# keep-starknet-strange/frieda

Measured on AMD Instinct MI355X. Metric: M31 field-elems/s committed (NTT+FRI+Merkle), higher is better.
Workload: dtype u32

## Files before the change

frieda_amd/csrc/context.cpp:

```cpp
#include <cstring>
#include <cstdlib>
#include <string.h>

#include <cstdio>

#include <algorithm>
#include <mutex>

#include "host.h"

extern char** environ;

namespace frieda {

static constexpr uint32_t IDX_MASK = 0x7fffffffu;

CPoint point_from_index(uint32_t index) {
    static const std::array<CPoint, 31> pow2 = [] {
        std::array<CPoint, 31> t{};
        CPoint cur{CIRCLE_GEN_X, CIRCLE_GEN_Y};
        for (auto& e : t) {
            e = cur;
            cur = cp_double(cur);
        }
        return t;
    }();
    CPoint res{1, 0};
    index &= IDX_MASK;
    for (uint32_t b = 0; index; b++, index >>= 1)
        if (index & 1u) res = cp_add(res, pow2[b]);
    return res;
}

Coset Coset::half_odds(uint32_t log_size) {
    Coset c;
    c.initial = 1u << (31 - (log_size + 2));
    c.step = log_size == 0 ? 0u : (1u << (31 - log_size));
    c.log_size = log_size;
    return c;
}
Coset Coset::doubled() const { return Coset{(initial * 2u) & IDX_MASK, (step * 2u) & IDX_MASK, log_size - 1}; }
uint32_t Coset::index_at(uint32_t i) const { return (initial + (uint32_t)((uint64_t)step * i)) & IDX_MASK; }
CPoint Coset::at(uint32_t i) const { return point_from_index(index_at(i)); }

Coset line_coset(uint32_t n, uint32_t m) {
    Coset c = Coset::half_odds(n - 1);
    while (c.log_size > m) c = c.doubled();
    return c;
}

CodecShape codec_shape(size_t len) {
    CodecShape s;
    s.n_felts = (8 * len + 29) / 30;
    uint32_t e = 2;
    while (((size_t)1 << e) < s.n_felts) e++;
    s.n_padded = (size_t)1 << e;
    s.log_size = e - 2;
    return s;
}

struct KernelTimerImpl {
    struct Span {
        const char* name;
        double alg_bytes;
        hipEvent_t start, stop;
    };
    std::vector<Span> spans;
    std::vector<hipEvent_t> pool;
    size_t used = 0;
    hipEvent_t next() {
        if (used == pool.size()) {
            hipEvent_t e;
            (void)hipEventCreate(&e);
            pool.push_back(e);
        }
        return pool[used++];
    }
    ~KernelTimerImpl() {
        for (auto e : pool) (void)hipEventDestroy(e);
    }
};

namespace k {
void timer_begin(KernelTimer* t, hipStream_t s, const char* name, double alg_bytes) {
    auto* ti = reinterpret_cast<KernelTimerImpl*>(t);
    KernelTimerImpl::Span sp{name, alg_bytes, ti->next(), ti->next()};
    (void)hipEventRecord(sp.start, s);
    ti->spans.push_back(sp);
}
void timer_end(KernelTimer* t, hipStream_t s) {
    auto* ti = reinterpret_cast<KernelTimerImpl*>(t);
    (void)hipEventRecord(ti->spans.back().stop, s);
}
}

k::Launch Ctx::launch() const {
    k::Launch l{stream, reinterpret_cast<k::KernelTimer*>(timer)};
    l.tune = &tuning;
    return l;
}

namespace k {
namespace {
struct KnobDesc {
    const char* name;
    long lo, hi;
    bool (*set)(Tuning&, long);
};
const KnobDesc KNOBS[] = {
    {"FRIEDA_T5_WIDE_LOG", 16, 24, [](Tuning& t, long v) { t.t5_wide_log = (uint32_t)v; return true; }},
    {"FRIEDA_T5_REG3_LOG", 0, 30, [](Tuning& t, long v) { t.t5_reg3_log = (uint32_t)v; return true; }},
    {"FRIEDA_T9_MAX_LOG", 8, 19, [](Tuning& t, long v) { t.t9_max_log = (uint32_t)v; return true; }},
    {"FRIEDA_TOP_MAX_LOG", 9, 11, [](Tuning& t, long v) { t.top_max_log = (uint32_t)v; return true; }},
    {"FRIEDA_NTT_CPW", 1, 4, [](Tuning& t, long v) {
         if (v == 4 && !t.lds_opt_in_ok) return false;
         t.ntt_cpw = (uint32_t)v;
         return true;
     }},
    {"FRIEDA_NTT_CPW_SMALL", 1, 4, [](Tuning& t, long v) { t.ntt_cpw_small = (uint32_t)v; return true; }},
    {"FRIEDA_NTT_REP", 0, 2, [](Tuning& t, long v) { t.ntt_rep = (uint32_t)v; return true; }},
    {"FRIEDA_NTT_NO_CP", 0, 1, [](Tuning& t, long v) { t.ntt_no_cp = v != 0; return true; }},
    {"FRIEDA_NTT_NO_PAD8", 0, 1, [](Tuning& t, long v) { t.ntt_no_pad8 = v != 0; return true; }},
    {"FRIEDA_NTT_PACKED_SRC", 0, 1, [](Tuning& t, long v) { t.ntt_packed_src = v != 0; return true; }},
    {"FRIEDA_NTT_TREE_REG_ONLY", 0, 1, [](Tuning& t, long v) { t.ntt_tree_reg_only = v != 0; return true; }},
    {"FRIEDA_NO_ENCODE_TREE_FUSION", 0, 1, [](Tuning& t, long v) { t.no_encode_tree_fusion = v != 0; return true; }},
    {"FRIEDA_ENCODE_TREE_FUSION_PROVE", 0, 1, [](Tuning& t, long v) { t.encode_tree_fusion_prove = v != 0; return true; }},
    {"FRIEDA_NO_SMALL_FUSED", 0, 1, [](Tuning& t, long v) { t.no_small_fused = v != 0; return true; }},
    {"FRIEDA_UNPACK_TILES", 1, 8, [](Tuning& t, long v) {
         if (v != 1 && v != 2 && v != 4 && v != 8) return false;
         t.unpack_tiles = (uint32_t)v;
         return true;
     }},
    {"FRIEDA_INTT_GENERIC", 0, 1, [](Tuning& t, long v) { t.intt_generic = v != 0; return true; }},
    {"FRIEDA_ERASURE_TREE_MIN_LOG", 6, 32, [](Tuning& t, long v) { t.erasure_tree_min_log = (uint32_t)v; return true; }},
    {"FRIEDA_TAIL_RUN_LOG", 4, 11, [](Tuning& t, long v) { t.tail_run_log = (uint32_t)v; return true; }},
    {"FRIEDA_HOST_DECOMMIT", 0, 1, [](Tuning& t, long v) { t.host_decommit = v != 0; return true; }},
    {"FRIEDA_GATHER_COPY", 0, 1, [](Tuning& t, long v) { t.gather_copy = v != 0; return true; }},
    {"FRIEDA_VERIFY_DEVICE_MIN", 0, 2147483648L, [](Tuning& t, long v) { t.verify_device_min = (uint32_t)v; return true; }},
    {"FRIEDA_VERIFY_SPLIT_MAX", 0, 2147483648L, [](Tuning& t, long v) { t.verify_split_max = (uint32_t)v; return true; }},
    {"FRIEDA_OPEN_SMALL_MAX", 0, 512, [](Tuning& t, long v) { t.open_small_max = (uint32_t)v; return true; }},
    {"FRIEDA_TREE_SKIP_LOG", 10, 40, [](Tuning& t, long v) { t.tree_skip_log = (uint32_t)v; return true; }},
    {"FRIEDA_TREE_SKIP_LONE_LOG", 10, 40, [](Tuning& t, long v) { t.tree_skip_lone_log = (uint32_t)v; return true; }},
    {"FRIEDA_SEEDS_FOLD_GROUP", 0, 64, [](Tuning& t, long v) { t.seeds_fold_group = (uint32_t)v; return true; }},
    {"FRIEDA_TP_MIN_WGS", 0, 1 << 30, [](Tuning& t, long v) { t.tp_min_wgs = (uint32_t)v; return true; }},
    {"FRIEDA_GRIND_FRONT_WGS", 0, 2048, [](Tuning& t, long v) { t.grind_front_wgs = (uint32_t)v; return true; }},
    {"FRIEDA_GRIND_ITERS", 0, 64, [](Tuning& t, long v) { t.grind_iters = (uint32_t)v; return true; }},
    {"FRIEDA_BATCH_BUDGET_MB", 0, 262144, [](Tuning& t, long v) { t.batch_budget_mb = (uint32_t)v; return true; }},
    {"FRIEDA_BATCH_CALLS_PER_CTX", 1, 64, [](Tuning& t, long v) { t.batch_calls_per_ctx = (uint32_t)v; return true; }},
};
}

bool tuning_set(Tuning& t, const char* name, long value) {
    if (!name) return false;
    for (const KnobDesc& k : KNOBS) {
        if (strcmp(k.name, name) == 0) {
            if (value < k.lo || value > k.hi) return false;
            return k.set(t, value);
        }
    }
    return false;
}

static const char* const PROCESS_VARS[] = {"FRIEDA_HIP_LIB", "FRIEDA_RCCL_PATH", "FRIEDA_MULTI_FORCE_RCCL", "FRIEDA_MULTI_NO_PREFETCH",
                                           "FRIEDA_MULTI_NO_NUMA_PIN", "FRIEDA_BENCH_FORCE_DIST", "FRIEDA_BENCH_CPU_THREADS", "FRIEDA_TEST_"};
static void warn_unknown_env_once() {
    static std::once_flag once;
    std::call_once(once, [] {
        for (char** e = ::environ; e && *e; e++) {
            if (strncmp(*e, "FRIEDA_", 7) != 0) continue;
            const char* eq = strchr(*e, '=');
            const size_t len = eq ? (size_t)(eq - *e) : strlen(*e);
            bool known = false;
            for (const KnobDesc& k : KNOBS) known = known || (strlen(k.name) == len && strncmp(k.name, *e, len) == 0);
            for (const char* pv : PROCESS_VARS) known = known || strncmp(pv, *e, strlen(pv)) == 0;
            if (!known) fprintf(stderr, "libfrieda_hip: note: environment variable %.*s is not an option of this library (ignored)\n", (int)len, *e);
        }
    });
}

Tuning tuning_from_env() {
    Tuning t;
    warn_unknown_env_once();
    for (const KnobDesc& k : KNOBS) {
        const char* e = getenv(k.name);
        if (!e) continue;
        char* end = nullptr;
        long v = strtol(e, &end, 10);
        if (end == e) v = 1;
        (void)tuning_set(t, k.name, v);
    }
    return t;
}

const Tuning& tuning_defaults() {
    static const Tuning d;
    return d;
}
}

int Ctx::set_kernel_timing(bool enabled) {
    if (enabled && !timer) timer = new KernelTimerImpl();
    if (!enabled && timer) {
        (void)hipStreamSynchronize(stream);
        delete timer;
        timer = nullptr;
    }
    return FRIEDA_OK;
}

std::string Ctx::kernel_timing_report(bool reset) {
    std::string out = "{\"kernels\": [";
    if (timer) {
        (void)hipStreamSynchronize(stream);
        struct Agg {
            const char* name;
            size_t launches;
            double ms, bytes;
        };
        std::vector<Agg> agg;
        for (auto& sp : timer->spans) {
            float ms = 0.f;
            if (hipEventElapsedTime(&ms, sp.start, sp.stop) != hipSuccess) continue;
            Agg* a = nullptr;
            for (auto& x : agg)
                if (strcmp(x.name, sp.name) == 0) a = &x;
            if (!a) {
                agg.push_back(Agg{sp.name, 0, 0.0, 0.0});
                a = &agg.back();
            }
            a->launches++;
            a->ms += ms;
            a->bytes += sp.alg_bytes;
        }
        bool first = true;
        for (auto& a : agg) {
            char buf[256];
            snprintf(buf, sizeof buf, "%s{\"name\": \"%s\", \"launches\": %zu, \"total_ms\": %.6f, \"alg_bytes\": %.1f}", first ? "" : ", ",
                     a.name, a.launches, a.ms, a.bytes);
            out += buf;
            first = false;
        }
        if (reset) {
            timer->spans.clear();
            timer->used = 0;
        }
    }
    out += "]}";
    return out;
}

int Ctx::fail(int code, const std::string& what) {
    err = what;
    return code;
}
int Ctx::hip_fail(hipError_t e, const char* what) {
    err = std::string(what) + ": " + hipGetErrorString(e);
    return FRIEDA_ERR_HIP;
}

int Ctx::ensure_arena(size_t bytes) {
    if (tuning.test_arena_limit && bytes > tuning.test_arena_limit) {
        err = "workspace of " + std::to_string(bytes) + " B refused by the test limit";
        return FRIEDA_ERR_NOMEM;
    }
    if (bytes <= arena_bytes) return FRIEDA_OK;
    if (arena) {
        FR_HIP(this, hipStreamSynchronize(stream));
        FR_HIP(this, hipFree(arena));
        arena = nullptr;
        arena_bytes = 0;
    }
    size_t want = (bytes + ((size_t)1 << 20) - 1) & ~(((size_t)1 << 20) - 1);
    hipError_t e = hipMalloc((void**)&arena, want);
// ... 103 lines not shown
```

frieda_amd/csrc/kernels.h:

```cpp
#pragma once
#include <hip/hip_runtime.h>
#include <stddef.h>
#include <stdint.h>

#include "field.h"

namespace frieda {
namespace k {

inline size_t tw_level_offset(uint32_t n, uint32_t lv) { return ((size_t)1 << (n - 1)) - ((size_t)1 << (n - 1 - lv)); }
__device__ __forceinline__ size_t tw_level_offset_dev(uint32_t n, uint32_t lv) {
    return ((size_t)1 << (n - 1)) - ((size_t)1 << (n - 1 - lv));
}

struct KernelTimer;
struct Tuning {
    uint32_t t5_wide_log = 18;
    uint32_t t5_reg3_log = 0;
    uint32_t t9_max_log = 17;
    uint32_t top_max_log = 9;
    uint32_t ntt_cpw = 4;
    uint32_t ntt_cpw_small = 1;
    uint32_t ntt_rep = 2;
    bool ntt_no_pad8 = false;
    bool ntt_packed_src = true;
    bool ntt_no_cp = false;
    bool ntt_tree_reg_only = false;
    bool no_encode_tree_fusion = false;
    bool encode_tree_fusion_prove = false;
    bool no_small_fused = false;
    uint32_t unpack_tiles = 4;
    bool intt_generic = false;
    uint32_t erasure_tree_min_log = 15;
    uint32_t tail_run_log = 9;
    bool host_decommit = false;
    bool gather_copy = false;
    uint32_t verify_device_min = 2;
    uint32_t verify_split_max = 256;
    uint32_t open_small_max = 512;
    uint32_t test_grind_first_log = 0;
    uint32_t batch_budget_mb = 0;
    uint32_t tree_skip_log = 18;
    uint32_t tree_skip_lone_log = 23;
    uint32_t tp_min_wgs = 768;
    uint32_t grind_iters = 0;
    uint32_t grind_front_wgs = 768;
    uint32_t seeds_fold_group = 0;
    uint32_t batch_calls_per_ctx = 1;
    uint64_t device_mem_bytes = 0;
    bool lds_opt_in_ok = true;
    uint64_t test_arena_limit = 0;
    uint64_t test_verify_pass_bytes = 0;
    uint64_t test_verify_scratch_bytes = 0;
    bool test_poison = false;
    uint32_t test_poison_word = 0;
};
inline uint32_t tree_skip_threshold(const Tuning& t, uint32_t batch) {
    return batch >= 2 ? t.tree_skip_log : (t.tree_skip_lone_log > t.tree_skip_log ? t.tree_skip_lone_log : t.tree_skip_log);
}
Tuning tuning_from_env();
bool tuning_set(Tuning& t, const char* name, long value);
const Tuning& tuning_defaults();

struct Launch {
    hipStream_t stream;
    KernelTimer* timer;
    uint32_t batch = 1;
    size_t bstride = 0;
    const Tuning* tune = &tuning_defaults();
};
void timer_begin(KernelTimer* t, hipStream_t s, const char* name, double alg_bytes);
void timer_end(KernelTimer* t, hipStream_t s);
struct Scope {
    const Launch& l;
    Scope(const Launch& l_, const char* name, double alg_bytes) : l(l_) {
        if (l.timer) timer_begin(l.timer, l.stream, name, alg_bytes * l.batch);
    }
    ~Scope() {
        if (l.timer) timer_end(l.timer, l.stream);
    }
};

struct DomainScalars {
    uint32_t init_x, init_y;
    uint32_t inv_init_x, inv_init_y;
};

void unpack30(const Launch& L, const uint8_t* d_bytes, size_t len, uint32_t* d_out, size_t n_out, size_t src_bstride = 0);

int blake2s_ceiling(hipStream_t s, uint32_t* d_scratch, double* leaf_per_s, double* node_per_s, double* clock = nullptr);
size_t blake2s_ceiling_scratch_bytes();

void bit_reverse_columns(const Launch& L, uint32_t* d_cols, size_t stride, uint32_t ncols, uint32_t log_size);

struct TwiddleSeeds {
    CPoint p0;
    CPoint step[32];
};
void gen_twiddles(const Launch& L, uint32_t n, const TwiddleSeeds& seeds, uint32_t* d_tw, uint32_t* d_itw, void* d_scratch8k);

void circle_evaluate(const Launch& L_, const uint32_t* d_coef, size_t coef_stride, uint32_t ncols, uint32_t L, uint32_t n,
                     const uint32_t* d_tw, DomainScalars ds, uint32_t* d_out, size_t out_stride);
void circle_evaluate_prefix(const Launch& L_, const uint32_t* d_coef, size_t coef_stride, uint32_t ncols, uint32_t L, uint32_t n, uint32_t out_log,
                            const uint32_t* d_tw, DomainScalars ds, uint32_t* d_out, size_t out_stride);

struct EncodeTreeSink {
    uint8_t* layers;
    uint8_t* last_out;
};
constexpr uint32_t ENCODE_TREE_LEVELS = 7;
hipError_t ntt_opt_in_dynamic_lds();
struct EncodeFoldSink {
    const uint32_t* itw;
    uint32_t alpha0[4], alpha1[4];
    bool accumulate;
    uint32_t* line1;
    uint32_t* line2;
};
bool circle_evaluate_fold2(const Launch& L_, const uint32_t* d_coef, size_t coef_stride, uint32_t L, uint32_t n, const uint32_t* d_tw,
                           DomainScalars ds, uint32_t* d_out, size_t out_stride, const EncodeFoldSink& fs, hipError_t* err);
struct BlobSource {
    const uint8_t* bytes;
    size_t len;
    size_t bstride;
    size_t n_padded;
};
uint32_t circle_evaluate_into_tree(const Launch& L_, const uint32_t* d_coef, size_t coef_stride, uint32_t ncols, uint32_t L, uint32_t n,
                               const uint32_t* d_tw, DomainScalars ds, uint32_t* d_out, size_t out_stride, const EncodeTreeSink* sink,
                               const BlobSource* blob = nullptr);

void circle_interpolate_block(const Launch& L_, const uint32_t* d_block, size_t in_stride, uint32_t ncols, uint32_t L, uint32_t n,
                              uint32_t block, const uint32_t* d_itw, DomainScalars ds, uint32_t* d_coef, size_t out_stride);
void cells_combine(const Launch& L_, const uint32_t* d_w, const uint32_t* d_vinv, uint32_t R, uint32_t ncols, uint32_t m, uint32_t* d_coef,
                   size_t coef_stride, size_t vinv_pitch = 0);
size_t cells_inverse_scratch_bytes(uint32_t R);
uint32_t* cells_inverse_index_buffer(uint8_t* d_scratch, uint32_t R);
void cells_matrix_inverse_device(const Launch& L_, const uint32_t* d_cell_index, uint32_t R, uint32_t j_bits, uint32_t m, uint32_t n,
                                 const uint32_t* d_tw, uint8_t* d_scratch, const uint32_t** d_vinv_out, size_t* pitch_out,
                                 const uint32_t** d_state_out);
void pack30(const Launch& L_, const uint32_t* d_felts, size_t n_felts, uint8_t* d_out, size_t len);

struct ErasureDomain {
    CPoint init;
    CPoint step_pow[32];
    uint32_t n;
};
void erasure_points(const Launch& L_, const ErasureDomain& g, const uint32_t* d_pos, uint32_t count, uint32_t* d_px, uint32_t* d_py);
void erasure_lines(const Launch& L_, const ErasureDomain& g, const uint32_t* d_pos, uint32_t n_lines, uint32_t* d_la, uint32_t* d_lb,
                   uint32_t* d_lc);
size_t erasure_zpart_chunks(uint32_t count, uint32_t n_lines);
void erasure_zeval(const Launch& L_, const uint32_t* d_px, const uint32_t* d_py, uint32_t count, const uint32_t* d_la, const uint32_t* d_lb,
                   const uint32_t* d_lc, uint32_t n_lines, bool own, uint32_t* d_zpart, uint32_t* d_z);
void erasure_known_weights(const Launch& L_, const uint32_t* d_px, const uint32_t* d_py, uint32_t count, uint32_t n, uint32_t* d_z);
void erasure_cellconst(const Launch& L_, const ErasureDomain& g, const uint32_t* d_cell_pos, uint32_t n_cells, uint32_t m, uint32_t* d_kc);
void erasure_zeval_cells(const Launch& L_, const uint32_t* d_px, uint32_t count, uint32_t m, const uint32_t* d_kc, uint32_t n_cells, bool own,
                         uint32_t* d_zpart, uint32_t* d_z);
void erasure_known_weights_cells(const Launch& L_, const uint32_t* d_px, uint32_t count, uint32_t n, uint32_t m, uint32_t* d_z);
size_t erasure_sample_lists_chunks(uint32_t n_cells);
hipError_t erasure_sample_lists(const Launch& L_, const uint32_t* d_idx, uint32_t n_cells, uint32_t domain_cells, uint32_t ncols, uint32_t log_cell,
                          uint32_t* d_owner, uint32_t* d_chunk_sum, uint32_t* d_chunk_off, uint32_t* d_first_cell, uint32_t* d_first_row,
                          uint32_t* d_state, uint32_t* d_pos, uint32_t* d_src);
void erasure_cell_firsts(const Launch& L_, const uint32_t* d_pos, uint32_t n_cells, uint32_t log_cell, uint32_t* d_out);
void erasure_lines32(const Launch& L_, const uint32_t* d_px128, const uint32_t* d_py128, const uint32_t* d_la, const uint32_t* d_lb, const uint32_t* d_lc,
                     uint32_t n_lines, uint32_t nodes, uint32_t* d_out);
void erasure_pairmul(const Launch& L_, const uint32_t* d_ext, uint32_t n_nodes, uint32_t size, uint32_t* d_out);
void erasure_ze(const Launch& L_, const ErasureDomain& g1, const uint32_t* d_zs, uint32_t count, uint32_t n, uint32_t* d_ze);
void erasure_fold_prefix(const Launch& L_, const uint32_t* d_in, size_t in_stride, uint32_t ncols, uint32_t out_log, uint32_t cnt, const uint32_t* d_tw,
                         uint32_t dom_n, uint32_t* d_out, size_t out_stride);
void erasure_gather(const Launch& L_, const uint32_t* d_src, const uint32_t* d_pos, uint32_t count, uint32_t* d_out);
void erasure_scatter(const Launch& L_, const uint32_t* d_cells, const uint32_t* d_src, const uint32_t* d_pos, const uint32_t* d_z, uint32_t count,
                     uint32_t ncols, uint32_t log_cell, uint32_t* d_w, size_t w_stride);
void erasure_divide(const Launch& L_, const uint32_t* d_ev, size_t ev_stride, const uint32_t* d_z, const uint32_t* d_px, uint32_t count, uint32_t ncols,
                    uint32_t n, uint32_t* d_block, size_t block_stride);
void erasure_check(const Launch& L_, const uint32_t* d_cells, const uint32_t* d_src, const uint32_t* d_pos, uint32_t count, uint32_t ncols,
                   uint32_t log_cell, const uint32_t* d_ev, size_t ev_stride, uint32_t* d_mismatch);

// ... 259 lines not shown
```

frieda_amd/csrc/ntt.hip:

```cpp
#include <hip/hip_runtime.h>

#include <type_traits>

#include <cstdlib>

#include "clock_stamps.h"
#include "kernels.h"
#include "tree_dev.h"

namespace frieda {
namespace k {

namespace {
using namespace treedev;

constexpr int NTT_THREADS = 256;
constexpr uint32_t TILE_LOG = 12;
#ifndef FRIEDA_NTT_PAD32
constexpr uint32_t TILE_WORDS = (1u << TILE_LOG) + (1u << (TILE_LOG - 4));
#else
constexpr uint32_t TILE_WORDS = (1u << TILE_LOG) + (1u << (TILE_LOG - 5));
#endif
constexpr uint32_t MAX_COLS_PER_WG = 4;
constexpr uint32_t MID_LOG_W = 4;
// ... 360 lines not shown
            const uint32_t lo = 8 - 4 * s;
            uint32_t* col = lds + pbase[s];
#pragma unroll
            for (int r = 0; r < 16; r++) x[r] = col[pad((uint32_t)r << lo)];
            radix16_stage(x, twd[s]);
            if (s + 1 < NS || LOG_W != 0) {
#pragma unroll
                for (int r = 0; r < 16; r++) col[pad((uint32_t)r << lo)] = x[r];
            }
            if (LOG_W == 0 && NS == 3 && s == 1)
                __builtin_amdgcn_wave_barrier();
            else
                __syncthreads();
        }
        uint32_t* dst = out + (size_t)c * a.out_stride;
        if (LOG_W == 0) {
            uint4* o = reinterpret_cast<uint4*>(dst + gbase + 16u * g);
            o[0] = make_uint4(x[0], x[1], x[2], x[3]);
            o[1] = make_uint4(x[4], x[5], x[6], x[7]);
            o[2] = make_uint4(x[8], x[9], x[10], x[11]);
            o[3] = make_uint4(x[12], x[13], x[14], x[15]);
        } else {
#pragma unroll
            for (int kk = 0; kk < 4; kk++) {
                const uint32_t e = piece_e(kk), p = pad(e);
                *reinterpret_cast<uint4*>(dst + global_of(e)) = make_uint4(lds[p], lds[p + 1], lds[p + 2], lds[p + 3]);
            }
            __syncthreads();
        }
    }
}

struct PackedBlob {
    const uint8_t* p;
    uint32_t full;
    uint32_t tail;
};
__device__ __forceinline__ PackedBlob packed_blob(const uint8_t* __restrict__ p, size_t len) {
    PackedBlob b{p, (uint32_t)(len >> 2), 0u};
    for (size_t i = 4 * (size_t)b.full; i < len; i++) b.tail |= (uint32_t)p[i] << (8 * (i & 3));
    return b;
}
__device__ __forceinline__ uint32_t packed_dword(const PackedBlob& b, uint32_t d) {
    const bool in = d < b.full;
    const uint32_t v = *reinterpret_cast<const uint32_t*>(b.p + ((in ? d : 0u) << 2));
    return in ? v : (d == b.full ? b.tail : 0u);
}
__device__ __forceinline__ uint32_t packed_felt(const PackedBlob& b, uint32_t f) {
    const uint32_t d = (15u * f) >> 4, sh = (30u * f) & 31u;
    const uint64_t pair = ((uint64_t)packed_dword(b, d + 1) << 32) | packed_dword(b, d);
    return (uint32_t)(pair >> sh) & 0x3fffffffu;
}

template <int COLS, bool PACKED>
__global__ __launch_bounds__(NTT_THREADS) void ntt_tile12_rep_kernel(NttArgs a) {
    ntt_enter();
    constexpr int NS = 2;
    constexpr uint32_t LOG_W = MID_LOG_W;
    __shared__ uint32_t lds[TILE_WORDS];
    const uint32_t g = threadIdx.x;
    const uint32_t nwb_log = a.i_lo - LOG_W;
    const uint32_t wblk = blockIdx.x & ((1u << nwb_log) - 1);
    const uint32_t hblk0 = (blockIdx.x >> nwb_log) << a.rep_log;
    constexpr uint32_t wmask = (1u << LOG_W) - 1;
    const size_t col0 = (size_t)blockIdx.y * COLS;
    uint32_t* out = a.out + col0 * a.out_stride + blockIdx.z * a.bstride_w;

    auto piece_e = [&](int kk) { return 4u * g + 1024u * (uint32_t)kk; };
    auto low_of = [&](uint32_t e) { return (wblk << LOG_W) | ((e >> LOG_W) << a.i_lo) | (e & wmask); };

    const uint32_t e0 = stage_group_base(g, 8);
    uint32_t src[COLS][16];
    if constexpr (PACKED) {
        const PackedBlob blob = packed_blob(a.pk + blockIdx.z * a.pk_bstride, a.pk_len);
#pragma unroll
        for (int c = 0; c < COLS; c++) {
#pragma unroll
            for (int r = 0; r < 16; r++) {
                const uint32_t idx = low_of(e0 | ((uint32_t)r << 8)) & a.in_mask;
                const bool ok = idx < a.in_limit;
                const uint32_t v = packed_felt(blob, ok ? (uint32_t)((col0 + c) * a.pk_col_felts) + idx : 0u);
                src[c][r] = ok ? v : 0u;
            }
        }
    } else {
#pragma unroll
        for (int c = 0; c < COLS; c++) {
#pragma unroll
            for (int r = 0; r < 16; r++) {
                const uint32_t idx = low_of(e0 | ((uint32_t)r << 8)) & a.in_mask;
                src[c][r] = idx < a.in_limit ? (a.in + col0 * a.in_stride + blockIdx.z * a.bstride_w)[(size_t)c * a.in_stride + idx] : 0u;
            }
        }
    }
    uint32_t pbase[NS];
#pragma unroll
    for (int s = 0; s < NS; s++) {
        const uint32_t lo = 8 - 4 * s;
        pbase[s] = pad(stage_group_base(g, lo));
    }

#pragma unroll 1
    for (uint32_t h = 0; h < (1u << a.rep_log); h++) {
        const uint32_t hblk = hblk0 + h;
        const uint32_t gbase = hblk << (a.i_hi + 1);
        uint32_t twd[NS][15];
#pragma unroll
        for (int s = 0; s < NS; s++) {
            const uint32_t lo = 8 - 4 * s;
            const uint32_t base = stage_group_base(g, lo);
#pragma unroll
            for (int q = 0; q < 4; q++) {
                const uint32_t b = lo + 3 - q;
                const uint32_t i = a.i_lo + b - LOG_W;
                const uint32_t hbase = (hblk << (a.i_hi - i)) | (base >> (b + 1));
                const uint32_t* lvl = a.tw + tw_level_offset_dev(a.n, i - 1) + hbase;
#pragma unroll
                for (int u = 0; u < (1 << q); u++) {
                    uint32_t v = lvl[u];
                    if (s == 0) v = (uint32_t)__builtin_amdgcn_readfirstlane((int)v);
                    twd[s][(1 << q) - 1 + u] = 2u * v;
                }
            }
        }
#pragma unroll
        for (int c = 0; c < COLS; c++) {
            uint32_t x[16];
#pragma unroll
            for (int r = 0; r < 16; r++) x[r] = src[c][r];
#pragma unroll
            for (int s = 0; s < NS; s++) {
                const uint32_t lo = 8 - 4 * s;
                uint32_t* col = lds + pbase[s];
                if (s > 0) {
#pragma unroll
                    for (int r = 0; r < 16; r++) x[r] = col[pad((uint32_t)r << lo)];
                }
                radix16_stage(x, twd[s]);
#pragma unroll
                for (int r = 0; r < 16; r++) col[pad((uint32_t)r << lo)] = x[r];
                __syncthreads();
            }
            uint32_t* dst = out + (size_t)c * a.out_stride + gbase;
#pragma unroll
            for (int kk = 0; kk < 4; kk++) {
                const uint32_t e = piece_e(kk), p = pad(e);
                *reinterpret_cast<uint4*>(dst + low_of(e)) = make_uint4(lds[p], lds[p + 1], lds[p + 2], lds[p + 3]);
            }
            __syncthreads();
        }
    }
}

struct NttTreeArgs {
    NttArgs a;
    uint8_t* layers;
    uint8_t* last_out;
    size_t bstride;
};


template <bool STORE_ALL>
__device__ __forceinline__ void last_pass_four_columns(const NttArgs& a, uint32_t* lds, uint32_t g, uint32_t hblk, const uint32_t* in, uint32_t* out,
                                                       uint32_t (&v)[4][16]) {
    const uint32_t gbase = hblk << TILE_LOG;
    uint32_t pbase[3];
    uint32_t twd[3][15];
#pragma unroll
    for (int s = 0; s < 3; s++) {
        const uint32_t lo = 8 - 4 * s;
        const uint32_t base = stage_group_base(g, lo);
        pbase[s] = pad(base);
#pragma unroll
        for (int q = 0; q < 4; q++) {
            const uint32_t b = lo + 3 - q;
            const uint32_t hbase = (hblk << (11 - b)) | (base >> (b + 1));
            if (s == 2 && q == 3) {
#pragma unroll
                for (int u = 0; u < 8; u++) twd[s][7 + u] = 2u * circle_twiddle(a.tw, a.n, hbase + (uint32_t)u, a.init_y);
            } else {
                const uint32_t* lvl = a.tw + tw_level_offset_dev(a.n, b - 1) + hbase;
#pragma unroll
                for (int u = 0; u < (1 << q); u++) {
                    uint32_t v = lvl[u];
                    if (s == 0) v = (uint32_t)__builtin_amdgcn_readfirstlane((int)v);
                    twd[s][(1 << q) - 1 + u] = 2u * v;
                }
            }
        }
    }
    auto piece_e = [&](int kk) { return 4u * g + 1024u * (uint32_t)kk; };

    uint4 pre[4];
#pragma unroll
    for (int kk = 0; kk < 4; kk++) pre[kk] = *reinterpret_cast<const uint4*>(in + ((gbase | piece_e(kk)) & a.in_mask));

#pragma unroll
    for (int c = 0; c < 4; c++) {
#pragma unroll
        for (int kk = 0; kk < 4; kk++) {
            const uint32_t p = pad(piece_e(kk));
            lds[p] = pre[kk].x;
            lds[p + 1] = pre[kk].y;
            lds[p + 2] = pre[kk].z;
            lds[p + 3] = pre[kk].w;
        }
        __syncthreads();
        if (c + 1 < 4) {
            const uint32_t* src = in + (size_t)(c + 1) * a.in_stride;
#pragma unroll
            for (int kk = 0; kk < 4; kk++) pre[kk] = *reinterpret_cast<const uint4*>(src + ((gbase | piece_e(kk)) & a.in_mask));
        }
#pragma unroll
        for (int s = 0; s < 3; s++) {
            const uint32_t lo = 8 - 4 * s;
            uint32_t* col = lds + pbase[s];
            uint32_t* x = v[c];
#pragma unroll
            for (int r = 0; r < 16; r++) x[r] = col[pad((uint32_t)r << lo)];
            radix16_stage<FRIEDA_NTT_GROUP_FUSED>(*reinterpret_cast<uint32_t(*)[16]>(x), twd[s]);
            if (s < 2) {
#pragma unroll
                for (int r = 0; r < 16; r++) col[pad((uint32_t)r << lo)] = x[r];
            }
            if (s == 1)
                __builtin_amdgcn_wave_barrier();
            else
                __syncthreads();
        }
        if (STORE_ALL) {
            uint4* o = reinterpret_cast<uint4*>(out + (size_t)c * a.out_stride + gbase + 16u * g);
            o[0] = make_uint4(v[c][0], v[c][1], v[c][2], v[c][3]);
            o[1] = make_uint4(v[c][4], v[c][5], v[c][6], v[c][7]);
            o[2] = make_uint4(v[c][8], v[c][9], v[c][10], v[c][11]);
            o[3] = make_uint4(v[c][12], v[c][13], v[c][14], v[c][15]);
        }
    }

}

FR_CLOCK_DECL(g_clock_ntt_last_tree)
template <bool STORE_ALL, bool REG_ONLY, bool TP>
__global__ __launch_bounds__(NTT_THREADS) void ntt_last_tree_kernel(NttTreeArgs A) {
    ntt_enter();
    __shared__ uint32_t lds[TILE_WORDS];
    __shared__ __attribute__((aligned(16))) uint32_t RC[8 * (256 + 4)];
    __shared__ __attribute__((aligned(16))) uint32_t RD[8 * (128 + 4)];
    const NttArgs& a = A.a;
    uint32_t g_tie = threadIdx.x;
    FR_CLOCK_BEGIN(g_tie)
    const uint32_t g = g_tie;
    const uint32_t hblk = blockIdx.x;
    const uint32_t gbase = hblk << TILE_LOG;
    const uint32_t* in = a.in + blockIdx.z * a.bstride_w;
    uint32_t* out = a.out + blockIdx.z * a.bstride_w;

    uint32_t v[4][16];
    last_pass_four_columns<STORE_ALL>(a, lds, g, hblk, in, out, v);

    const uint32_t m = a.n;
    uint8_t* layers = A.layers + blockIdx.z * A.bstride;
    uint8_t* out_b = STORE_ALL ? layers + layer_off(m, m - 1) : nullptr;
    uint8_t* out_c = STORE_ALL ? layers + layer_off(m, m - 2) : nullptr;
    uint8_t* out_d = STORE_ALL ? layers + layer_off(m, m - 3) : nullptr;
    uint8_t* out_e = STORE_ALL ? layers + layer_off(m, m - 4) : (REG_ONLY ? A.last_out + blockIdx.z * A.bstride : nullptr);
    const size_t leaf0 = (size_t)gbase + 16u * g;
    uint32_t hprev[8], hdprev[8];
#pragma unroll 1
    for (int it = 0; it < 4; it++) {
        const size_t l0 = leaf0 + 4u * (uint32_t)it;
        uint32_t hb[2][8];
        auto half_ab = [&](auto half_c) {
            constexpr int half = decltype(half_c)::value;
            uint32_t ha[2][8];
            leaf_hash<TP ? FRIEDA_B2_IDLE_NTT_LEAF : B2_LAT>(v[0][2 * half], v[1][2 * half], v[2][2 * half], v[3][2 * half], ha[0]);
            leaf_hash<TP ? FRIEDA_B2_IDLE_NTT_LEAF : B2_LAT>(v[0][2 * half + 1], v[1][2 * half + 1], v[2][2 * half + 1], v[3][2 * half + 1], ha[1]);
            uint32_t mm[16];
#pragma unroll
            for (int w = 0; w < 8; w++) mm[w] = ha[0][w], mm[8 + w] = ha[1][w];
            b2_merkle_block<TP ? FRIEDA_B2_IDLE_NTT_NODE : B2_LAT>(mm, hb[half]);
        };
        half_ab(std::integral_constant<int, 0>{});
        half_ab(std::integral_constant<int, 1>{});
        if (STORE_ALL) {
            store_hash(out_b, l0 >> 1, hb[0]);
            store_hash(out_b, (l0 >> 1) + 1, hb[1]);
        }
        uint32_t hc[8];
        {
            uint32_t mm[16];
#pragma unroll
            for (int w = 0; w < 8; w++) mm[w] = hb[0][w], mm[8 + w] = hb[1][w];
            b2_merkle_block<TP ? FRIEDA_B2_IDLE_NTT_NODE : B2_LAT>(mm, hc);
        }
        if (STORE_ALL) store_hash(out_c, l0 >> 2, hc);
        if ((it & 1) == 0) {
#pragma unroll
            for (int w = 0; w < 8; w++) hprev[w] = hc[w];
        } else {
            uint32_t hd[8], mm[16];
#pragma unroll
            for (int w = 0; w < 8; w++) mm[w] = hprev[w], mm[8 + w] = hc[w];
            b2_merkle_block<TP ? FRIEDA_B2_IDLE_NTT_NODE : B2_LAT>(mm, hd);
            if (STORE_ALL) store_hash(out_d, l0 >> 3, hd);
            if (it == 1) {
#pragma unroll
// ... 178 lines not shown
    }
    {
        uint4* o = reinterpret_cast<uint4*>(a.out + (size_t)c * a.out_stride + gbase + 16u * g);
        o[0] = make_uint4(x[0], x[1], x[2], x[3]);
        o[1] = make_uint4(x[4], x[5], x[6], x[7]);
        o[2] = make_uint4(x[8], x[9], x[10], x[11]);
        o[3] = make_uint4(x[12], x[13], x[14], x[15]);
        uint32_t* mine = lds + pad(16u * g);
#pragma unroll
        for (int r = 0; r < 16; r++) mine[r] = x[r];
    }
    __syncthreads();
    const uint32_t T = threadIdx.x, n = a.n;
    const size_t e0 = (size_t)gbase + 4u * T;
    uint32_t v[4][4];
#pragma unroll
    for (int cc = 0; cc < 4; cc++) {
        const uint32_t* t4 = cp_lds + cc * TILE_WORDS + pad(4u * T);
#pragma unroll
        for (int k = 0; k < 4; k++) v[cc][k] = t4[k];
    }
    const QM31Mat am0 = qm_matrix({A.alpha0[0], A.alpha0[1], A.alpha0[2], A.alpha0[3]});
    const QM31Mat am1 = qm_matrix({A.alpha1[0], A.alpha1[1], A.alpha1[2], A.alpha1[3]});
    const size_t i0 = e0 >> 1;
    const uint2 xy = *reinterpret_cast<const uint2*>(A.itw + 2 * (i0 >> 2));
    const uint32_t it0 = (i0 & 2) ? m31_neg(xy.x) : xy.y, it1 = (i0 & 2) ? xy.x : m31_neg(xy.y);
    const uint32_t il = A.itw[e0 >> 2];
    QM31 l1[2];
    l1[0] = qm_fold_pair(QM31{v[0][0], v[1][0], v[2][0], v[3][0]}, QM31{v[0][1], v[1][1], v[2][1], v[3][1]}, it0, am0);
    l1[1] = qm_fold_pair(QM31{v[0][2], v[1][2], v[2][2], v[3][2]}, QM31{v[0][3], v[1][3], v[2][3], v[3][3]}, it1, am0);
    const size_t s1 = (size_t)1 << (n - 1), s2 = (size_t)1 << (n - 2);
    uint32_t* d1 = A.line1 + i0;
    if (ACC) {
        const QM31 al = {A.alpha0[0], A.alpha0[1], A.alpha0[2], A.alpha0[3]};
        const QM31 asq = qm_mul(al, al);
        uint2 o[4];
#pragma unroll
        for (int cc = 0; cc < 4; cc++) o[cc] = *reinterpret_cast<const uint2*>(d1 + cc * s1);
        l1[0] = qm_add(qm_mul(QM31{o[0].x, o[1].x, o[2].x, o[3].x}, asq), l1[0]);
        l1[1] = qm_add(qm_mul(QM31{o[0].y, o[1].y, o[2].y, o[3].y}, asq), l1[1]);
    }
    *reinterpret_cast<uint2*>(d1) = make_uint2(l1[0].a, l1[1].a);
    *reinterpret_cast<uint2*>(d1 + s1) = make_uint2(l1[0].b, l1[1].b);
    *reinterpret_cast<uint2*>(d1 + 2 * s1) = make_uint2(l1[0].c, l1[1].c);
    *reinterpret_cast<uint2*>(d1 + 3 * s1) = make_uint2(l1[0].d, l1[1].d);
    const QM31 l2 = qm_fold_pair(l1[0], l1[1], il, am1);
    uint32_t* d2 = A.line2 + (e0 >> 2);
    d2[0] = l2.a;
    d2[s2] = l2.b;
    d2[2 * s2] = l2.c;
    d2[3 * s2] = l2.d;
}

}

FR_CLOCK_READER(frieda_debug_clock_ntt_last_tree, g_clock_ntt_last_tree)

namespace {
uint32_t evaluate_plan(const Launch& L_, const uint32_t* d_coef, size_t coef_stride, uint32_t ncols, uint32_t L, uint32_t n, uint32_t out_log,
                       const uint32_t* d_tw, DomainScalars ds, uint32_t* d_out, size_t out_stride, const EncodeTreeSink* sink,
                       const EncodeFoldSink* fsink = nullptr, const BlobSource* blob = nullptr);
}

void circle_evaluate(const Launch& L_, const uint32_t* d_coef, size_t coef_stride, uint32_t ncols, uint32_t L, uint32_t n,
                     const uint32_t* d_tw, DomainScalars ds, uint32_t* d_out, size_t out_stride) {
    (void)evaluate_plan(L_, d_coef, coef_stride, ncols, L, n, n, d_tw, ds, d_out, out_stride, nullptr);
}

void circle_evaluate_prefix(const Launch& L_, const uint32_t* d_coef, size_t coef_stride, uint32_t ncols, uint32_t L, uint32_t n, uint32_t out_log,
                            const uint32_t* d_tw, DomainScalars ds, uint32_t* d_out, size_t out_stride) {
    (void)evaluate_plan(L_, d_coef, coef_stride, ncols, L, n, out_log < L ? L : (out_log > n ? n : out_log), d_tw, ds, d_out, out_stride, nullptr);
}

uint32_t circle_evaluate_into_tree(const Launch& L_, const uint32_t* d_coef, size_t coef_stride, uint32_t ncols, uint32_t L, uint32_t n,
                               const uint32_t* d_tw, DomainScalars ds, uint32_t* d_out, size_t out_stride, const EncodeTreeSink* sink,
                               const BlobSource* blob) {
    return evaluate_plan(L_, d_coef, coef_stride, ncols, L, n, n, d_tw, ds, d_out, out_stride, sink, nullptr, blob);
}

hipError_t ntt_opt_in_dynamic_lds() {
    const int bytes = (int)(MAX_COLS_PER_WG * TILE_WORDS * sizeof(uint32_t));
    hipError_t e = hipFuncSetAttribute(reinterpret_cast<const void*>(ntt_tile_kernel), hipFuncAttributeMaxDynamicSharedMemorySize, bytes);
    if (e != hipSuccess) return e;
    e = hipFuncSetAttribute(reinterpret_cast<const void*>(ntt_last_fold_cp_kernel<false>), hipFuncAttributeMaxDynamicSharedMemorySize, bytes);
    if (e != hipSuccess) return e;
    return hipFuncSetAttribute(reinterpret_cast<const void*>(ntt_last_fold_cp_kernel<true>), hipFuncAttributeMaxDynamicSharedMemorySize, bytes);
}

bool circle_evaluate_fold2(const Launch& L_, const uint32_t* d_coef, size_t coef_stride, uint32_t L, uint32_t n, const uint32_t* d_tw,
                           DomainScalars ds, uint32_t* d_out, size_t out_stride, const EncodeFoldSink& fs, hipError_t* err) {
    *err = hipSuccess;
    if (evaluate_plan(L_, d_coef, coef_stride, 4, L, n, n, d_tw, ds, d_out, out_stride, nullptr, &fs)) return true;
    if (!fs.accumulate) {
        *err = hipMemsetAsync(fs.line1, 0, sizeof(uint32_t) * ((size_t)4 << (n - 1)), L_.stream);
        if (*err != hipSuccess) return false;
    }
    fold_circle_into_line(L_, fs.line1, (size_t)1 << (n - 1), d_out, out_stride, n, fs.itw, ds, Alpha{{fs.alpha0[0], fs.alpha0[1], fs.alpha0[2], fs.alpha0[3]}});
    fold_line(L_, fs.line1, (size_t)1 << (n - 1), n - 1, n, fs.itw, ds, Alpha{{fs.alpha1[0], fs.alpha1[1], fs.alpha1[2], fs.alpha1[3]}}, fs.line2,
              (size_t)1 << (n - 2));
    return false;
}

namespace {
uint32_t evaluate_plan(const Launch& L_, const uint32_t* d_coef, size_t coef_stride, uint32_t ncols, uint32_t L, uint32_t n, uint32_t out_log,
                       const uint32_t* d_tw, DomainScalars ds, uint32_t* d_out, size_t out_stride, const EncodeTreeSink* sink,
                       const EncodeFoldSink* fsink, const BlobSource* blob) {
    const size_t N = (size_t)1 << out_log;
    hipStream_t s = L_.stream;
    bool blob_pending = blob != nullptr;
    auto unpack_now = [&]() {
        unpack30(L_, blob->bytes, blob->len, const_cast<uint32_t*>(d_coef), blob->n_padded, blob->bstride);
        blob_pending = false;
    };
    const double enc_bytes = 4.0 * ncols * ((double)N + (double)((size_t)1 << L));
    if (L == 0) {
        if (blob_pending) unpack_now();
        Scope scope(L_, "ntt_broadcast", enc_bytes);
        dim3 grid((unsigned)((N + 255) / 256), ncols, L_.batch);
        ntt_broadcast_kernel<<<grid, 256, 0, s>>>(d_coef, coef_stride, d_out, out_stride, N, L_.bstride / 4);
        return 0;
    }
    const uint32_t cpw_max = L_.tune->ntt_cpw <= MAX_COLS_PER_WG ? L_.tune->ntt_cpw : MAX_COLS_PER_WG;
    uint32_t cpw = cpw_max;
    while (ncols % cpw) cpw--;
    const size_t lds_bytes = (size_t)cpw * TILE_WORDS * sizeof(uint32_t);

    const uint32_t last_t = L < TILE_LOG ? L : TILE_LOG;
    uint32_t rest = L - last_t;
    const uint32_t mid_max = TILE_LOG - MID_LOG_W;
    const uint32_t n_mid_generic = (rest + mid_max - 1) / mid_max;
    uint32_t n_mid_fast = 0;
    NttArgs a{};
    a.in = d_coef;
    a.in_stride = coef_stride;
    a.in_mask = (uint32_t)(((size_t)1 << L) - 1);
    a.out = d_out;
    a.out_stride = out_stride;
    a.tw = d_tw;
    a.n = n;
    a.init_y = ds.init_y;
    a.bstride_w = L_.bstride / 4;
    uint32_t cpw4 = MAX_COLS_PER_WG;
    const uint32_t cpw_small = L_.tune->ntt_cpw_small;
    if ((N >> TILE_LOG) * (size_t)L_.batch < 512) cpw4 = cpw_small;
    while (ncols % cpw4) cpw4--;
    uint32_t fused_levels = 0;
    auto launch_pass = [&](uint32_t t, const char* name) {
        const bool aligned = ((a.in_stride | a.out_stride) & 3) == 0 && (a.in_mask & 3u) == 3u &&
                             ((reinterpret_cast<uintptr_t>(a.in) | reinterpret_cast<uintptr_t>(a.out) | L_.bstride) & 15) == 0;
        const uint32_t hb_log = n - 1 - a.i_hi;
        const uint64_t rep_wgs = (uint64_t)((N >> TILE_LOG) >> (hb_log < 3 ? hb_log : 3)) * (ncols / 2) * L_.batch;
        const bool use_rep = L_.tune->ntt_rep == 1 || (L_.tune->ntt_rep == 2 && rep_wgs >= 1024);
        const bool rep = use_rep && out_log == n && aligned && t == 8 && a.log_w == MID_LOG_W && hb_log >= 1 && ((uint64_t)a.in_mask >> (a.i_hi + 1)) == 0 && ncols % 2 == 0;
        bool packed = false;
        if (blob_pending) {
            packed = rep && L_.tune->ntt_packed_src && blob->len >= 4 && blob->len <= ((size_t)1 << 30) &&
                     (uint64_t)ncols * coef_stride <= ((uint64_t)1 << 28) && (reinterpret_cast<uintptr_t>(blob->bytes) & 3) == 0 &&
                     (L_.batch == 1 || (blob->bstride & 3) == 0);
            if (packed)
                blob_pending = false;
            else
                unpack_now();
        }
        if (sink && aligned && a.log_w == 0 && t == 12 && ncols == 4 && n >= TILE_LOG && out_log == n) {
            NttTreeArgs ta{};
            ta.a = a;
            ta.a.ncols = 4;
            ta.layers = sink->layers;
            ta.last_out = sink->last_out;
            ta.bstride = L_.bstride;
            const bool reg_only = L_.tune->ntt_tree_reg_only;
            const uint32_t levels = reg_only ? 5u : ENCODE_TREE_LEVELS;
            double bytes = enc_bytes / ((n_mid_fast ? n_mid_fast : n_mid_generic) + 1) + 48.0 * (double)N;
            for (uint32_t l = 1; l < levels; l++) bytes += 96.0 * (double)(N >> l);
            Scope scope(L_, reg_only ? "ntt_last_tree5" : "ntt_last_tree7", bytes);
            const dim3 grid((unsigned)(N >> TILE_LOG), 1, L_.batch);
            const bool tp = (size_t)grid.x * grid.z >= L_.tune->tp_min_wgs;
#define FR_LAUNCH_LAST_TREE(SA, RO)                                                      \
    do {                                                                                 \
        if (tp)                                                                          \
            ntt_last_tree_kernel<SA, RO, true><<<grid, NTT_THREADS, 0, s>>>(ta);         \
        else                                                                             \
            ntt_last_tree_kernel<SA, RO, false><<<grid, NTT_THREADS, 0, s>>>(ta);        \
    } while (0)
            if (sink->layers && reg_only)
                FR_LAUNCH_LAST_TREE(true, true);
            else if (sink->layers)
                FR_LAUNCH_LAST_TREE(true, false);
            else if (reg_only)
                FR_LAUNCH_LAST_TREE(false, true);
            else
                FR_LAUNCH_LAST_TREE(false, false);
#undef FR_LAUNCH_LAST_TREE
            fused_levels = levels;
            return;
        }
        if (fsink && aligned && a.log_w == 0 && t == 12 && ncols == 4 && n >= TILE_LOG + 2 && out_log == n && L_.batch == 1 &&
            ((reinterpret_cast<uintptr_t>(fsink->line1) | reinterpret_cast<uintptr_t>(fsink->line2) | reinterpret_cast<uintptr_t>(fsink->itw)) & 15) == 0) {
            NttFoldArgs fa{};
            fa.a = a;
            fa.a.ncols = 4;
            fa.itw = fsink->itw;
            fa.inv_init_y = ds.inv_init_y;
            for (int i = 0; i < 4; i++) fa.alpha0[i] = fsink->alpha0[i], fa.alpha1[i] = fsink->alpha1[i];
            fa.line1 = fsink->line1;
            fa.line2 = fsink->line2;
            Scope scope(L_, "ntt_last_fold2", enc_bytes / ((n_mid_fast ? n_mid_fast : n_mid_generic) + 1) + 36.0 * (double)N);
            const dim3 grid((unsigned)(N >> TILE_LOG), 1, 1);
            const bool side_by_side = (N >> TILE_LOG) < 512 && L_.tune->lds_opt_in_ok && L_.tune->ntt_cpw == 4 && !L_.tune->ntt_no_cp;
            const size_t cp_lds = (size_t)4 * TILE_WORDS * sizeof(uint32_t);
            if (side_by_side && fsink->accumulate)
                ntt_last_fold_cp_kernel<true><<<grid, NTT_CP_THREADS, cp_lds, s>>>(fa);
            else if (side_by_side)
                ntt_last_fold_cp_kernel<false><<<grid, NTT_CP_THREADS, cp_lds, s>>>(fa);
            else if (fsink->accumulate)
                ntt_last_fold_kernel<true><<<grid, NTT_THREADS, 0, s>>>(fa);
            else
                ntt_last_fold_kernel<false><<<grid, NTT_THREADS, 0, s>>>(fa);
            fused_levels = 1;
            return;
        }
        Scope scope(L_, name, enc_bytes / ((n_mid_fast ? n_mid_fast : n_mid_generic) + 1));
        if (rep) {
            a.rep_log = hb_log < 3 ? hb_log : 3;
            a.ncols = 2;
            dim3 grid((unsigned)((N >> TILE_LOG) >> a.rep_log), ncols / 2, L_.batch);
            if (packed) {
                a.pk = blob->bytes;
                a.pk_len = blob->len;
                a.pk_bstride = L_.batch > 1 ? blob->bstride : 0;
                a.pk_col_felts = coef_stride;
                ntt_tile12_rep_kernel<2, true><<<grid, NTT_THREADS, 0, s>>>(a);
            } else {
                ntt_tile12_rep_kernel<2, false><<<grid, NTT_THREADS, 0, s>>>(a);
            }
            a.rep_log = 0;
        } else if (aligned && t + a.log_w == TILE_LOG && (t == 12 || t == 8 || t == 4)) {
            a.ncols = cpw4;
            dim3 grid((unsigned)(N >> TILE_LOG), ncols / cpw4, L_.batch);
            if (t == 12)
                ntt_tile12_kernel<3, 0><<<grid, NTT_THREADS, 0, s>>>(a);
            else if (t == 8)
                ntt_tile12_kernel<2, MID_LOG_W><<<grid, NTT_THREADS, 0, s>>>(a);
            else
                ntt_tile12_kernel<1, 8><<<grid, NTT_THREADS, 0, s>>>(a);
        } else {
            a.ncols = cpw;
            set_stages(a, t);
            dim3 grid((unsigned)(N >> (t + a.log_w)), ncols / cpw, L_.batch);
            ntt_tile_kernel<<<grid, NTT_THREADS, lds_bytes, s>>>(a);
        }
    };
    a.in_limit = a.in_mask + 1;
    uint32_t i_hi = L - 1;
    const bool no_pad8 = L_.tune->ntt_no_pad8;
    const uint32_t units = (rest + 3) / 4, padz = 4 * units - rest;
    const bool base_aligned = ((a.in_stride | a.out_stride) & 3) == 0 &&
                              ((reinterpret_cast<uintptr_t>(a.in) | reinterpret_cast<uintptr_t>(a.out) | L_.bstride) & 15) == 0;
    if (rest > 0 && base_aligned && padz <= out_log - L && L >= 4 && (!no_pad8 || (padz == 0 && (units & 1) == 0))) {
        n_mid_fast = (units + 1) / 2;
        uint32_t top = L - 1 + padz, left = units;
        bool first = true;
        while (left) {
            const uint32_t t = (left & 1) ? 4u : 8u;
            a.i_hi = top;
            a.i_lo = top + 1 - t;
            a.log_w = TILE_LOG - t;
            if (first) {
                a.in_mask = (uint32_t)(((size_t)1 << (L + padz)) - 1);
                a.in_limit = (uint32_t)1 << L;
            }
            launch_pass(t, "ntt_pass_mid");
            a.in = d_out;
            a.in_stride = out_stride;
            a.in_mask = (uint32_t)(N - 1);
            a.in_limit = (uint32_t)N;
            top -= t;
            left -= t / 4;
            first = false;
        }
        rest = 0;
        i_hi = last_t - 1;
    }
    const uint32_t n_mid = n_mid_generic;
    for (uint32_t p = 0; p < n_mid && rest; p++) {
        uint32_t t = (rest + (n_mid - p) - 1) / (n_mid - p);
        a.i_hi = i_hi;
        a.i_lo = i_hi + 1 - t;
        a.log_w = t >= mid_max ? MID_LOG_W : TILE_LOG - t;
        launch_pass(t, "ntt_pass_mid");
        a.in = d_out;
        a.in_stride = out_stride;
        a.in_mask = (uint32_t)(N - 1);
        a.in_limit = (uint32_t)N;
        rest -= t;
        i_hi = a.i_lo - 1;
    }
    a.i_hi = i_hi;
    a.i_lo = 0;
    a.log_w = 0;
    launch_pass(last_t, "ntt_pass_last");
    return fused_levels;
}
}

}
}
```

Measured before the change: 48.79 billion.

## Add 8K-element tile13 replicated NTT kernel with 32-wide full-line stores

Adds a new middle-pass NTT kernel that widens the contiguous column run from 16 to 32 words and doubles the LDS tile to 2^13 elements. Each thread now processes two 16-point groups, so every output store covers full 128-byte cache lines. It is selected by default through a new tuning knob when outputs are 128-byte aligned and there are enough workgroups. The goal is better write coalescing and fewer partial-line memory transactions, at the cost of more registers, larger LDS use, fewer workgroups and a different twiddle indexing scheme.

```diff
diff --git a/frieda_amd/csrc/context.cpp b/frieda_amd/csrc/context.cpp
--- a/frieda_amd/csrc/context.cpp
+++ b/frieda_amd/csrc/context.cpp
@@ -119,6 +119,7 @@
      }},
     {"FRIEDA_NTT_CPW_SMALL", 1, 4, [](Tuning& t, long v) { t.ntt_cpw_small = (uint32_t)v; return true; }},
     {"FRIEDA_NTT_REP", 0, 2, [](Tuning& t, long v) { t.ntt_rep = (uint32_t)v; return true; }},
+    {"FRIEDA_NTT_REP_LOGW", 4, 5, [](Tuning& t, long v) { t.ntt_rep_logw = (uint32_t)v; return true; }},
     {"FRIEDA_NTT_NO_CP", 0, 1, [](Tuning& t, long v) { t.ntt_no_cp = v != 0; return true; }},
     {"FRIEDA_NTT_NO_PAD8", 0, 1, [](Tuning& t, long v) { t.ntt_no_pad8 = v != 0; return true; }},
     {"FRIEDA_NTT_PACKED_SRC", 0, 1, [](Tuning& t, long v) { t.ntt_packed_src = v != 0; return true; }},
diff --git a/frieda_amd/csrc/kernels.h b/frieda_amd/csrc/kernels.h
--- a/frieda_amd/csrc/kernels.h
+++ b/frieda_amd/csrc/kernels.h
@@ -22,6 +22,7 @@
     uint32_t ntt_cpw = 4;
     uint32_t ntt_cpw_small = 1;
     uint32_t ntt_rep = 2;
+    uint32_t ntt_rep_logw = 5;
     bool ntt_no_pad8 = false;
     bool ntt_packed_src = true;
     bool ntt_no_cp = false;
diff --git a/frieda_amd/csrc/ntt.hip b/frieda_amd/csrc/ntt.hip
--- a/frieda_amd/csrc/ntt.hip
+++ b/frieda_amd/csrc/ntt.hip
@@ -536,6 +536,122 @@
     }
 }
 
+constexpr uint32_t LINE_LOG_W = 5;
+constexpr uint32_t LINE_TILE_LOG = 13;
+#ifndef FRIEDA_NTT_PAD32
+constexpr uint32_t LINE_TILE_WORDS = (1u << LINE_TILE_LOG) + (1u << (LINE_TILE_LOG - 4));
+#else
+constexpr uint32_t LINE_TILE_WORDS = (1u << LINE_TILE_LOG) + (1u << (LINE_TILE_LOG - 5));
+#endif
+__device__ __forceinline__ uint32_t line_group_base(uint32_t g, uint32_t j, int stage) {
+    if (stage == 0) return g | (j << 8);
+    const uint32_t hi = g >> 4;
+#ifndef FRIEDA_NTT_PAD32
+    const uint32_t half = (j ^ hi) & 1u;
+#else
+    const uint32_t half = j;
+#endif
+    return (hi << 9) | (half << 4) | (g & 15u);
+}
+
+template <int COLS, bool PACKED>
+__global__ __launch_bounds__(NTT_THREADS, 4) void ntt_tile13_rep_kernel(NttArgs a) {
+    ntt_enter();
+    constexpr uint32_t LOG_W = LINE_LOG_W;
+    __shared__ uint32_t lds[LINE_TILE_WORDS];
+    const uint32_t g = threadIdx.x;
+    const uint32_t nwb_log = a.i_lo - LOG_W;
+    const uint32_t wblk = blockIdx.x & ((1u << nwb_log) - 1);
+    const uint32_t hblk0 = (blockIdx.x >> nwb_log) << a.rep_log;
+    constexpr uint32_t wmask = (1u << LOG_W) - 1;
+    const size_t col0 = (size_t)blockIdx.y * COLS;
+    uint32_t* out = a.out + col0 * a.out_stride + blockIdx.z * a.bstride_w;
+
+    auto piece_e = [&](int kk) { return 4u * g + 1024u * (uint32_t)kk; };
+    auto low_of = [&](uint32_t e) { return (wblk << LOG_W) | ((e >> LOG_W) << a.i_lo) | (e & wmask); };
+
+    uint32_t pbase[2][2];
+#pragma unroll
+    for (int s = 0; s < 2; s++) {
+#pragma unroll
+        for (int j = 0; j < 2; j++) pbase[s][j] = pad(line_group_base(g, j, s));
+    }
+    PackedBlob blob{};
+    if constexpr (PACKED) blob = packed_blob(a.pk + blockIdx.z * a.pk_bstride, a.pk_len);
+
+#pragma unroll 1
+    for (int c = 0; c < COLS; c++) {
+        uint32_t src[2][16];
+        uint32_t gs = g;
+        asm volatile("" : "+v"(gs));
+        const uint32_t* in_c = a.in + (col0 + c) * a.in_stride + blockIdx.z * a.bstride_w;
+        const uint32_t felt0 = (uint32_t)((col0 + c) * a.pk_col_felts);
+#pragma unroll
+        for (int j = 0; j < 2; j++) {
+#pragma unroll
+            for (int r = 0; r < 16; r++) {
+                const uint32_t idx = low_of(line_group_base(gs, j, 0) | ((uint32_t)r << 9)) & a.in_mask;
+                const bool ok = idx < a.in_limit;
+                const uint32_t v = PACKED ? packed_felt(blob, ok ? felt0 + idx : 0u) : in_c[ok ? idx : 0u];
+                src[j][r] = ok ? v : 0u;
+            }
+            if constexpr (PACKED) {
+                uint32_t(&w)[16] = src[0];
+                if (j == 0)
+                    asm volatile("" : "+v"(gs), "+v"(w[0]), "+v"(w[1]), "+v"(w[2]), "+v"(w[3]), "+v"(w[4]), "+v"(w[5]), "+v"(w[6]), "+v"(w[7]), "+v"(w[8]),
+                                 "+v"(w[9]), "+v"(w[10]), "+v"(w[11]), "+v"(w[12]), "+v"(w[13]), "+v"(w[14]), "+v"(w[15]));
+            }
+        }
+#pragma unroll 1
+        for (uint32_t h = 0; h < (1u << a.rep_log); h++) {
+            const uint32_t hblk = hblk0 + h;
+            const uint32_t gbase = hblk << (a.i_hi + 1);
+            uint32_t twd[2][15];
+#pragma unroll
+            for (int s = 0; s < 2; s++) {
+                const uint32_t lo = 9 - 4 * s;
+                const uint32_t base = line_group_base(g, 0, s);
+#pragma unroll
+                for (int q = 0; q < 4; q++) {
+                    const uint32_t b = lo + 3 - q;
+                    const uint32_t i = a.i_lo + b - LOG_W;
+                    const uint32_t hbase = (hblk << (a.i_hi - i)) | (base >> (b + 1));
+                    const uint32_t* lvl = a.tw + tw_level_offset_dev(a.n, i - 1) + hbase;
+#pragma unroll
+                    for (int u = 0; u < (1 << q); u++) {
+                        uint32_t v = lvl[u];
+                        if (s == 0) v = (uint32_t)__builtin_amdgcn_readfirstlane((int)v);
+                        twd[s][(1 << q) - 1 + u] = 2u * v;
+                    }
+                }
+            }
+#pragma unroll
+            for (int s = 0; s < 2; s++) {
+                const uint32_t lo = 9 - 4 * s;
+#pragma unroll
+                for (int j = 0; j < 2; j++) {
+                    uint32_t* col = lds + pbase[s][j];
+                    uint32_t x[16];
+#pragma unroll
+                    for (int r = 0; r < 16; r++) x[r] = s == 0 ? src[j][r] : col[pad((uint32_t)r << lo)];
+                    radix16_stage(x, twd[s]);
+#pragma unroll
+                    for (int r = 0; r < 16; r++) col[pad((uint32_t)r << lo)] = x[r];
+                    __builtin_amdgcn_sched_barrier(0);
+                }
+                __syncthreads();
+            }
+            uint32_t* dst = out + (size_t)c * a.out_stride + gbase;
+#pragma unroll
+            for (int kk = 0; kk < 8; kk++) {
+                const uint32_t e = piece_e(kk), p = pad(e);
+                *reinterpret_cast<uint4*>(dst + low_of(e)) = make_uint4(lds[p], lds[p + 1], lds[p + 2], lds[p + 3]);
+            }
+            __syncthreads();
+        }
+    }
+}
+
 struct NttTreeArgs {
     NttArgs a;
     uint8_t* layers;
@@ -1020,6 +1136,8 @@
         const uint64_t rep_wgs = (uint64_t)((N >> TILE_LOG) >> (hb_log < 3 ? hb_log : 3)) * (ncols / 2) * L_.batch;
         const bool use_rep = L_.tune->ntt_rep == 1 || (L_.tune->ntt_rep == 2 && rep_wgs >= 1024);
         const bool rep = use_rep && out_log == n && aligned && t == 8 && a.log_w == MID_LOG_W && hb_log >= 1 && ((uint64_t)a.in_mask >> (a.i_hi + 1)) == 0 && ncols % 2 == 0;
+        const bool line_aligned = ((a.out_stride * 4) & 127) == 0 && ((reinterpret_cast<uintptr_t>(a.out) | L_.bstride) & 127) == 0;
+        const bool line = rep && L_.tune->ntt_rep_logw == 5 && line_aligned && (L_.tune->ntt_rep == 1 || rep_wgs >= 2048);
         bool packed = false;
         if (blob_pending) {
             packed = rep && L_.tune->ntt_packed_src && blob->len >= 4 && blob->len <= ((size_t)1 << 30) &&
@@ -1092,13 +1210,18 @@
         if (rep) {
             a.rep_log = hb_log < 3 ? hb_log : 3;
             a.ncols = 2;
-            dim3 grid((unsigned)((N >> TILE_LOG) >> a.rep_log), ncols / 2, L_.batch);
+            dim3 grid((unsigned)((N >> (line ? LINE_TILE_LOG : TILE_LOG)) >> a.rep_log), ncols / 2, L_.batch);
             if (packed) {
                 a.pk = blob->bytes;
                 a.pk_len = blob->len;
                 a.pk_bstride = L_.batch > 1 ? blob->bstride : 0;
                 a.pk_col_felts = coef_stride;
-                ntt_tile12_rep_kernel<2, true><<<grid, NTT_THREADS, 0, s>>>(a);
+                if (line)
+                    ntt_tile13_rep_kernel<2, true><<<grid, NTT_THREADS, 0, s>>>(a);
+                else
+                    ntt_tile12_rep_kernel<2, true><<<grid, NTT_THREADS, 0, s>>>(a);
+            } else if (line) {
+                ntt_tile13_rep_kernel<2, false><<<grid, NTT_THREADS, 0, s>>>(a);
             } else {
                 ntt_tile12_rep_kernel<2, false><<<grid, NTT_THREADS, 0, s>>>(a);
             }
```

Measured after the change: 48.93 billion, median of 6. About the same (+0.3%).
